# smolGura/fish-tts

Measured on AMD Instinct MI355X. Metric: semantic tokens/sec, higher is better.
Workload: dtype bf16; 1 GPU; openaudio-s1-mini shapes (BASELINE configs[1]): batch=1 per GPU, 48-token prompt, 215 frames (10 s), top-p sampling, hipGraph-captured frame step, + DAC codec decode; prompt_len=48, parallelism=replica x1, frame_engine=3

## Files before the change

fish-tts_amd/csrc/ar_kernels.h:

```cpp
#pragma once
#include "common.h"

namespace ft {

enum { PRO_NONE = 0, PRO_RMSNORM = 1 };
enum { EPI_STORE = 0, EPI_RESID = 1, EPI_SWIGLU = 2 };

__device__ __host__ __forceinline__ size_t xo_index(int m, int k, int ldm) { return ((size_t)(k >> 3) * ldm + m) * 8 + (k & 7); }

struct GemvP {
    const void* W;
    const void* bias;
    const float* x;
    int ldx;
    const void* gain;
    float eps;
    float* out;
    int ldo;
    const float* resid;
    int ldr;
    int N, K;
    int pro, epi;
    int nt;
};
// ... 1416 lines not shown
        const float* qrow = nullptr;
        if (p.noise && nfv < p.noise_rows) qrow = p.noise + (size_t)nfv * p.noise_row_len + p.noise_off;
        float q4[4];
        draw_noise4(p, ctl, qrow, i0, nfv, m, V, q4);
        ArgMax best{-1.f, 0x7fffffff};
#pragma unroll
        for (int e = 0; e < 4; ++e) {
            if (i0 + e < V) {
                const float prob = keep[e] ? rb<ROUND>(et[e] / Z2) : 0.f;
                best = better(best, ArgMax{rb<ROUND>(prob / rb<ROUND>(q4[e])), i0 + e});
            }
        }
        winner = block_best(best).i;
    }
    __syncthreads();
    finish_draw<WT>(p, m, winner, nfv);
}

struct SampCut {
    unsigned kstar;
    int nk;
    int all_kept;
    int argmax;
    float Lmax, Mt, Z2, Tc;
};

struct SampBigP {
    SampP s;
    SampCut* cut;
    int* chunk_cnt;
    float* part_score;
    int* part_idx;
    int nchunk;
};

__device__ __forceinline__ float key16_value(unsigned k16) {
    const uint32_t k = k16 << 16;
    const uint32_t u = (k & 0x80000000u) ? (k & 0x7fffffffu) : ~(k | 0xffffu);
    return __uint_as_float(u);
}

constexpr int SAMP_TH_THREADS = 1024;
constexpr int SAMP_TH_ROW = 33;
constexpr int SAMP_TH_OVF = 8;
constexpr size_t SAMP_TH_LDS = (size_t)SAMP_TH_THREADS * SAMP_TH_ROW * 4;

struct SampThShared {
    float red[16];
    int redi[16];
    float wsum[16];
    int wact[16];
    int AL[1024];
    unsigned ovf_key[SAMP_TH_OVF];
    unsigned ovf_cnt[SAMP_TH_OVF];
    int ovf_n;
    SampCut cut_s;
};

__device__ __forceinline__ void samp_cut_from_image(const SampBigP& b, const int m, const uint32_t* cimg, SampThShared& sh,
                                                    const bool has, const int kmax_t) {
    const SampP& p = b.s;
    const int tid = threadIdx.x, lane = tid & 63, wave = tid >> 6;
    const RowCtl ctl = p.ctl[m];
    float* red = sh.red;
    int* redi = sh.redi;
    float* wsum = sh.wsum;
    int* wact = sh.wact;
    int* AL = sh.AL;
    unsigned* ovf_key = sh.ovf_key;
    unsigned* ovf_cnt = sh.ovf_cnt;
    int& ovf_n = sh.ovf_n;
    SampCut& cut_s = sh.cut_s;
    const unsigned long long hb = __ballot(has);
    if (lane == 0) wact[wave] = __popcll(hb);
    __syncthreads();
    int abase = 0, n_active = 0;
    for (int w = 0; w < 16; ++w) { if (w < wave) abase += wact[w]; n_active += wact[w]; }
    if (has) AL[abase + __popcll(hb & ((1ull << lane) - 1ull))] = tid;
    ArgMax km = block_argmax(ArgMax{(float)kmax_t, tid}, red, redi);
    const unsigned kmax = (unsigned)(int)km.v;
    const float Lmax = key16_value(kmax);
    const int n_items = n_active * 64;
    const int ipt = (n_items + 1023) / 1024;
    const int i0 = tid * ipt, i1 = min(i0 + ipt, n_items);
    auto item_count = [&](int i, unsigned& k) -> float {
        const int g = AL[i >> 6], j = i & 63;
        k = 64u * g + j;
        const uint32_t w = cimg[g * SAMP_TH_ROW + (j >> 1)];
        unsigned c = (j & 1) ? (w >> 16) : (w & 0xffffu);
        if (c == 65535u)
            for (int q = 0; q < ovf_n && q < SAMP_TH_OVF; ++q) if (ovf_key[q] == k) c = ovf_cnt[q];
        return (float)c;
    };
    float z = 0.f;
    for (int i = i0; i < i1; ++i) {
        unsigned k;
        const float c = item_count(i, k);
        if (c > 0.f) z = fmaf(c, expf(key16_value(k) - Lmax), z);
    }
    const float Z = block_sum(z, red);
    const float tp = round_bf16(ctl.top_p);
    auto removed = [&](float cum) { return round_bf16(cum) > tp; };
    auto prob = [&](unsigned k16) { return round_bf16(expf(key16_value(k16) - Lmax) / Z); };
    float mt = 0.f;
    for (int i = i0; i < i1; ++i) {
        unsigned k;
        const float c = item_count(i, k);
        if (c > 0.f) mt = fmaf(c, prob(k), mt);
    }
    float suf = mt;
#pragma unroll
    for (int o = 1; o < 64; o <<= 1) {
        const float t = __shfl_down(suf, o, 64);
        if (lane + o < 64) suf += t;
    }
    __syncthreads();
    if (lane == 0) wsum[wave] = suf;
    __syncthreads();
    float above = suf - mt;
    for (int w = wave + 1; w < 16; ++w) above += wsum[w];
    int found = -1;
    unsigned f_key = 0;
    float f_above = 0.f, f_cnt = 0.f;
    float run = above;
    for (int i = i1 - 1; i >= i0; --i) {
        unsigned k;
        const float c = item_count(i, k);
        if (c > 0.f) {
            const float nxt = fmaf(c, prob(k), run);
            if (found < 0 && removed(nxt)) { found = i; f_key = k; f_above = run; f_cnt = c; }
            run = nxt;
        }
    }
    ArgMax who = block_argmax(ArgMax{found >= 0 ? (float)tid : -1.f, tid}, red, redi);
    if (tid == 0) { cut_s.all_kept = who.v < 0.f ? 1 : 0; cut_s.kstar = 0; cut_s.nk = 0; }
    __syncthreads();
    if (who.v >= 0.f && tid == (int)who.v) {
        const float pk = prob(f_key);
        int lo_n = 0, hi_n = (int)f_cnt;
        while (lo_n < hi_n) {
            const int mid = (lo_n + hi_n + 1) >> 1;
            if (removed(fmaf((float)mid, pk, f_above))) hi_n = mid - 1; else lo_n = mid;
        }
        if (f_key == kmax && lo_n < 1) lo_n = 1;
        cut_s.kstar = f_key;
        cut_s.nk = lo_n;
    }
    __syncthreads();
    const unsigned kstar = cut_s.kstar;
    const int nk = cut_s.nk, all_kept = cut_s.all_kept;
    const float Tc = fmaxf(ctl.temperature, 1e-5f);
    const float Mt = round_bf16(Lmax / Tc);
    float z2 = 0.f;
    for (int i = i0; i < i1; ++i) {
        unsigned k;
        const float c = item_count(i, k);
        if (c > 0.f) {
            float n = 0.f;
            if (all_kept || k > kstar) n = c;
            else if (k == kstar) n = (float)nk;
            if (n > 0.f) z2 = fmaf(n, expf(round_bf16(key16_value(k) / Tc) - Mt), z2);
        }
    }
    const float Z2 = block_sum(z2, red);
    if (tid == 0) {
        SampCut o;
        o.kstar = kstar; o.nk = nk; o.all_kept = all_kept; o.argmax = 0;
        o.Lmax = Lmax; o.Mt = Mt; o.Z2 = Z2; o.Tc = Tc;
        b.cut[m] = o;
    }
}

static __global__ __launch_bounds__(1024) void samp_cut_kernel(SampBigP b) {
    extern __shared__ __attribute__((aligned(16))) uint32_t cimg[];
    __shared__ SampThShared sh;
    __shared__ int pen_id[32];
    __shared__ float pen_val[32];
    const SampP& p = b.s;
    const int m = blockIdx.x, tid = threadIdx.x;
    float* L = p.logits + (size_t)m * p.ldl;
    const int V = p.V;
    const RowCtl ctl = p.ctl[m];
    const int nfv = p.nf[m];
    const int R = p.ncb + 1;
    const int* seq = p.seq + (size_t)m * R * p.cap;
    for (int i = tid; i < SAMP_TH_THREADS * SAMP_TH_ROW; i += 1024) cimg[i] = 0u;
    if (tid == 0) sh.ovf_n = 0;
    const int npen = nfv > 0 ? (p.cb == 0 ? R : 16) : 0;
    auto count1 = [&](float v) {
        const unsigned k = order_key(v) >> 16;
        atomicAdd(&cimg[(k >> 6) * SAMP_TH_ROW + ((k & 63u) >> 1)], (k & 1u) ? 0x10000u : 1u);
    };
    {
        if (nfv > 0) {
            const int it = nfv - 1;
            const int ws = it < 16 ? 0 : it - 16;
            if (tid < npen) {
                const int id = p.cb == 0 ? seq[(size_t)tid * p.cap + ws + 1] : seq[(size_t)(p.cb + 1) * p.cap + ws + 1 + tid];
                pen_id[tid] = -1;
                if (id >= 0 && id < V) {
                    const float sv = L[id];
                    pen_id[tid] = id;
                    pen_val[tid] = sv < 0.f ? round_bf16(sv * ctl.rep) : round_bf16(sv / ctl.rep);
                }
            }
            __syncthreads();
            if (tid < npen && pen_id[tid] >= 0) L[pen_id[tid]] = pen_val[tid];
        }
        if (p.cb == 0 && ctl.ban_eos && tid == 0 && p.im_end < V) L[p.im_end] = -INFINITY;
        __syncthreads();
        const int V16 = ((reinterpret_cast<uintptr_t>(L) & 15) == 0) ? (V / 16384) * 16384 : 0;
        float4 fa[4], fb[4];
        auto ld16 = [&](float4 (&f)[4], int base) {
#pragma unroll
            for (int u = 0; u < 4; ++u) f[u] = *reinterpret_cast<const float4*>(L + base + u * 4096 + tid * 4);
        };
        auto cnt16 = [&](const float4 (&f)[4]) {
#pragma unroll
            for (int u = 0; u < 4; ++u) { count1(f[u].x); count1(f[u].y); count1(f[u].z); count1(f[u].w); }
        };
        if (V16 > 0) ld16(fa, 0);
        for (int base = 0; base < V16; base += 32768) {
            if (base + 16384 < V16) ld16(fb, base + 16384);
            cnt16(fa);
            if (base + 32768 < V16) ld16(fa, base + 32768);
            if (base + 16384 < V16) cnt16(fb);
        }
        for (int base = V16; base < V; base += 4096) {
            float f[4];
#pragma unroll
            for (int u = 0; u < 4; ++u) { const int i = base + u * 1024 + tid; f[u] = i < V ? L[i] : 0.f; }
#pragma unroll
            for (int u = 0; u < 4; ++u) if (base + u * 1024 + tid < V) count1(f[u]);
        }
    }
    __syncthreads();
    const uint32_t* row = cimg + tid * SAMP_TH_ROW;
    int kmax_t = -1;
    unsigned tot = 0;
#pragma unroll 8
    for (int j = 0; j < 32; ++j) {
        const uint32_t w = row[j];
        const unsigned c0 = w & 0xffffu, c1 = w >> 16;
        if (c0) kmax_t = 64 * tid + 2 * j;
        if (c1) kmax_t = 64 * tid + 2 * j + 1;
        tot += c0 + c1;
    }
    const int total = (int)block_sum((float)tot, sh.red);
    if (total != V) {
        __shared__ unsigned exc_key[SAMP_TH_OVF];
        __shared__ unsigned exc_cnt[SAMP_TH_OVF];
        for (int i = tid; i < SAMP_TH_THREADS * SAMP_TH_ROW; i += 1024) cimg[i] = 0u;
        if (tid < SAMP_TH_OVF) { exc_key[tid] = 0xffffffffu; exc_cnt[tid] = 0u; }
        __syncthreads();
        for (int i = tid; i < V; i += 1024) {
            const unsigned k = order_key(L[i]) >> 16;
            uint32_t* d = &cimg[(k >> 6) * SAMP_TH_ROW + ((k & 63u) >> 1)];
            const unsigned shft = (k & 1u) * 16u;
            for (;;) {
                const uint32_t old = *reinterpret_cast<volatile uint32_t*>(d);
                if (((old >> shft) & 0xffffu) == 65535u) {
                    for (int q = 0; q < SAMP_TH_OVF; ++q) {
                        const unsigned prev = atomicCAS(&exc_key[q], 0xffffffffu, k);
                        if (prev == 0xffffffffu || prev == k) { atomicAdd(&exc_cnt[q], 1u); break; }
                    }
                    break;
                }
                if (atomicCAS(d, old, old + (1u << shft)) == old) break;
            }
        }
        __syncthreads();
        if (tid == 0) {
            int n = 0;
            for (int q = 0; q < SAMP_TH_OVF; ++q)
                if (exc_key[q] != 0xffffffffu) { sh.ovf_key[n] = exc_key[q]; sh.ovf_cnt[n] = 65535u + exc_cnt[q]; ++n; }
            sh.ovf_n = n;
        }
        kmax_t = -1;
        tot = 0;
        for (int j = 0; j < 32; ++j) {
            const uint32_t w = row[j];
            if (w & 0xffffu) kmax_t = 64 * tid + 2 * j;
            if (w >> 16) kmax_t = 64 * tid + 2 * j + 1;
            tot += (w & 0xffffu) + (w >> 16);
        }
        __syncthreads();
    }
    samp_cut_from_image(b, m, cimg, sh, tot != 0u, kmax_t);
}

static __global__ __launch_bounds__(256) void samp_count_kernel(SampBigP b) {
    __shared__ float red[4];
    const SampP& p = b.s;
    const int m = blockIdx.y, tid = threadIdx.x;
    const int c0 = blockIdx.x * 1024;
    const float* L = p.logits + (size_t)m * p.ldl;
    const SampCut cut = b.cut[m];
    float c = 0.f;
#pragma unroll
    for (int e = 0; e < 4; ++e) {
        const int i = c0 + 4 * tid + e;
        if (i < p.V && (order_key(L[i]) >> 16) == cut.kstar) c += 1.f;
    }
    c = wave_sum(c);
    if ((tid & 63) == 0) red[tid >> 6] = c;
    __syncthreads();
    if (tid == 0) b.chunk_cnt[(size_t)m * b.nchunk + blockIdx.x] = (int)(red[0] + red[1] + red[2] + red[3]);
}

static __global__ __launch_bounds__(256) void samp_race_kernel(SampBigP b) {
    __shared__ float red[4];
    __shared__ int redi[4];
    __shared__ int wcnt[4];
    const SampP& p = b.s;
    const int m = blockIdx.y, tid = threadIdx.x, lane = tid & 63, wave = tid >> 6;
    const int c0 = blockIdx.x * 1024;
    const float* L = p.logits + (size_t)m * p.ldl;
    const int V = p.V;
    const RowCtl ctl = p.ctl[m];
    const int nfv = p.nf[m];
    const SampCut cut = b.cut[m];
    float basef = 0.f;
// ... 72 lines not shown
```

fish-tts_amd/csrc/engine.h:

```cpp
#pragma once
#include <hip/hip_runtime.h>

#include <map>
#include <string>
#include <vector>

#include "../../include/fishtts_hip.h"
#include "../../include/fishtts_hip_test.h"
#include "common.h"

namespace ft {
struct RowCtl;
struct SampCut;
struct EngLayer;
}

struct FtTensor {
    void* p = nullptr;
    std::vector<int64_t> shape;
    int dtype = FT_BF16;
    int64_t numel() const {
        int64_t n = 1;
        for (auto s : shape) n *= s;
        return n;
// ... 31 lines not shown
          *femb = nullptr, *xf = nullptr, *qkvf = nullptr, *gf = nullptr, *flog = nullptr, *part_o = nullptr,
          *part_ml = nullptr;
    int n_slots = 0, nsplit = 1, cap = 0, fastV = 0, y_ld = 0;
    int nsplit_max = 1;
    bool nsplit_fixed = false;
    float *pf_x = nullptr, *pf_qkv = nullptr, *pf_y = nullptr;
    ft::bf16_t *pf_xn = nullptr, *pf_ybf = nullptr, *pf_g = nullptr, *pf_qbf = nullptr;
    int4* pf_seqs = nullptr;
    int2* pf_rows = nullptr;
    ft::bf16_t *xo_x = nullptr, *xo_xf = nullptr, *xo_femb = nullptr, *xo_y = nullptr, *xo_g = nullptr;
    ft::bf16_t* wide_qkv0_tab = nullptr;
    int xo_ldm = 0;
    int xo_pair = 0;
    bool no_attn_wide = false;
    bool no_head_stream = false;
    bool no_pair = false;
    int wide_min = 5;
    bool wide_ok = false;
    bool prefill_v0 = false;
    int prefill_gemm_mode = 2;
    size_t cache_m_stride = 0, fcache_m_stride = 0;

    int *d_pos = nullptr, *d_tok = nullptr, *d_tokn = nullptr, *d_seq = nullptr, *d_nf = nullptr,
        *d_done = nullptr, *d_prompt = nullptr;
    ft::RowCtl* d_ctl = nullptr;
    int *h_pin = nullptr;
    float* noise = nullptr;
    long noise_rows = 0, noise_row_len = 0;

    ft::SampCut* samp_cut = nullptr;
    int* samp_chunk_cnt = nullptr;
    float* samp_part_score = nullptr;
    int* samp_part_idx = nullptr;

    bool eng_on = false;
    bool eng_fast_on = false;
    int eng_nb = 0;
    ft::EngLayer *eng_layers = nullptr, *eng_flayers = nullptr;
    unsigned *eng_gx = nullptr, *eng_gqkv = nullptr, *eng_gy = nullptr, *eng_gxb = nullptr, *eng_gg = nullptr;
    unsigned long long* eng_gpart = nullptr;
    unsigned* eng_fast_g = nullptr;
    unsigned* eng_ctl = nullptr;
    size_t eng_lds_slow = 0, eng_lds_fast = 0, eng_fast_words = 0, eng_pool_words = 0;
    bool eng_relay = true;
    void* eng_qkv0_tab = nullptr;
    bool eng_pair = false;
    bool xl_shape = false;
    bool eng_xl = false;
    std::string path_str;
    const void* eng_slow_fn = nullptr;
    const void* eng_fast_fn = nullptr;
    size_t eng_pool_bytes = 0, eng_gpart_bytes = 0, eng_fast_bytes = 0;
    bool eng_suspended = false;
    int eng_strikes = 0, eng_last_where = 0;
    bool eng_owner = false;
    std::string eng_why;

    std::map<int, hipGraphExec_t> graphs;
    std::map<int, int> graph_nodes;

    bool prof = false, prof_count_only = false;
    std::vector<hipEvent_t> prof_ev;
    int64_t prof_bytes = 0, prof_launches = 0;

    CodecState* codec = nullptr;
};
// ... 15 lines not shown
```

fish-tts_amd/csrc/engine.hip:

```cpp
#include "engine.h"
#include "ar_kernels.h"
#include "frame_engine.h"
#include "wide_kernels.h"
#include "codec_kernels.h"

#include <math.h>

#include <algorithm>
#include <mutex>
#include <stdio.h>
#include <stdlib.h>
#include <string.h>

using namespace ft;

static std::string g_create_err;
static void eng_release(ft_ctx* ctx);

ft_status ft_fail(ft_ctx* ctx, ft_status code, const std::string& msg) {
    if (ctx) ctx->err = msg; else g_create_err = msg;
    return code;
}

template <typename S, typename D>
// ... 157 lines not shown
        const size_t S = c.max_seq_len;
        FT_TRY(dmalloc(ctx, &ctx->pf_x, S * c.dim));
        FT_TRY(dmalloc(ctx, &ctx->pf_qkv, S * qkvN));
        FT_TRY(dmalloc(ctx, &ctx->pf_y, S * c.n_head * c.head_dim));
        FT_TRY(dmalloc(ctx, &ctx->pf_xn, S * c.dim));
        FT_TRY(dmalloc(ctx, &ctx->pf_ybf, S * c.n_head * c.head_dim));
        FT_TRY(dmalloc(ctx, &ctx->pf_g, S * c.intermediate_size));
        FT_TRY(dmalloc(ctx, &ctx->pf_qbf, S * c.n_head * c.head_dim));
        FT_TRY(dmalloc(ctx, &ctx->pf_seqs, M));
        FT_TRY(dmalloc(ctx, &ctx->pf_rows, S));
    }
    if (c.dtype == FT_F16 || !ctx->prefill_v0) {
        const int HD = c.n_head * c.head_dim, HDf = c.fast_n_head * c.fast_head_dim;
        ctx->wide_ok = !getenv("FT_NO_WIDE") && !c.fast_attention_qkv_bias && !c.fast_attention_o_bias && c.fast_dim == c.dim &&
                       wide_k_ok(c.dim) && wide_k_ok(HD) && wide_k_ok(c.intermediate_size) && wide_k_ok(HDf) && wide_k_ok(c.fast_intermediate_size) &&
                       qkvN % 32 == 0 && fqkvN % 32 == 0 && c.intermediate_size % 16 == 0 && c.fast_intermediate_size % 16 == 0 &&
                       c.dim % 16 == 0 && c.vocab_size % 32 == 0 && ctx->fastV % 16 == 0;
        if (ctx->wide_ok) {
            ctx->xo_pair = (int)((M + 15) / 16 * 16);
            ctx->no_pair = getenv("FT_NO_PAIR") != nullptr;
            ctx->no_attn_wide = getenv("FT_NO_ATTN_WIDE") != nullptr;
            ctx->no_head_stream = getenv("FT_NO_HEAD_STREAM") != nullptr;
            ctx->xo_ldm = 2 * ctx->xo_pair;
            const size_t P = ctx->xo_ldm;
            FT_TRY(dmalloc(ctx, &ctx->xo_x, P * c.dim));
            FT_TRY(dmalloc(ctx, &ctx->xo_xf, P * c.fast_dim));
            FT_TRY(dmalloc(ctx, &ctx->xo_femb, P * c.fast_dim));
            FT_TRY(dmalloc(ctx, &ctx->xo_y, P * (size_t)std::max(HD, HDf)));
            FT_TRY(dmalloc(ctx, &ctx->xo_g, P * (size_t)std::max(c.intermediate_size, c.fast_intermediate_size)));
        }
    }
    const size_t nchunk = ((size_t)c.vocab_size + 1023) / 1024;
    FT_TRY(dmalloc(ctx, &ctx->samp_cut, M));
    FT_TRY(dmalloc(ctx, &ctx->samp_chunk_cnt, M * nchunk));
    FT_TRY(dmalloc(ctx, &ctx->samp_part_score, M * nchunk));
    FT_TRY(dmalloc(ctx, &ctx->samp_part_idx, M * nchunk));
    FT_HIP(ctx, hipHostMalloc((void**)&ctx->h_pin, (3 * M + 8) * sizeof(int), hipHostMallocDefault));
    return FT_OK;
}

extern "C" ft_status ft_create(const ft_ar_config* ar, const ft_codec_config* codec, int32_t device, ft_ctx** out) {
    if (!out || (!ar && !codec)) return ft_fail(nullptr, FT_ERR_ARG, "ft_create: need a config and an out pointer");
    int ndev = 0;
    if (hipGetDeviceCount(&ndev) != hipSuccess || ndev == 0)
        return ft_fail(nullptr, FT_ERR_HIP, "ft_create: no HIP device visible (the MI355X path has no CPU fallback)");
    if (device < 0 || device >= ndev) return ft_fail(nullptr, FT_ERR_ARG, "ft_create: bad device index");
    ft_ctx* ctx = new ft_ctx();
    ctx->device = device;
    ft_status st = FT_OK;
    do {
        if (hipSetDevice(device) != hipSuccess) { st = ft_fail(ctx, FT_ERR_HIP, "hipSetDevice failed"); break; }
        if (hipStreamCreateWithFlags(&ctx->stream, hipStreamNonBlocking) != hipSuccess) {
            st = ft_fail(ctx, FT_ERR_HIP, "hipStreamCreate failed"); break;
        }
        if (ar) {
            ctx->c = *ar;
            ctx->has_ar = true;
            if ((st = ar_validate(ctx)) != FT_OK) break;
            if ((st = ar_alloc(ctx)) != FT_OK) break;
            ar_expected(ctx);
        }
        if (codec) {
            ctx->cc = *codec;
            ctx->has_codec = true;
            if ((st = codec_create(ctx)) != FT_OK) break;
            codec_expected(ctx);
// ... 893 lines not shown
    else { s.logits = ctx->flog + (size_t)m0 * ctx->fastV; s.ldl = ctx->fastV; s.V = ctx->fastV; }
    s.ctl = ctx->d_ctl + m0; s.tokn = ctx->d_tokn + (size_t)m0 * R; s.seq = ctx->d_seq + (size_t)m0 * R * ctx->cap;
    s.cap = ctx->cap; s.nf = ctx->d_nf + m0; s.cb = cb; s.ncb = c.num_codebooks; s.sem_begin = c.semantic_begin_id;
    s.im_end = c.im_end_id; s.cbsize = c.codebook_size; s.fast_emb = ctx->fast_emb;
    s.femb = ctx->femb + (size_t)m0 * c.fast_dim; s.Df = c.fast_dim; s.noise = ctx->noise;
    s.noise_row_len = ctx->noise_row_len; s.noise_rows = ctx->noise_rows;
    s.noise_off = cb == 0 ? 0 : (long)c.vocab_size + (long)(cb - 1) * ctx->fastV;
    s.last = last ? 1 : 0; s.tok = ctx->d_tok + (size_t)m0 * R; s.pos = ctx->d_pos + m0; s.done = ctx->d_done + m0;
    if (wide_batch(L)) {
        s.femb_xo = (cb == 0 && wide_pair(L) ? ctx->xo_x + (size_t)ctx->xo_pair * 8 : ctx->xo_femb) + (size_t)m0 * 8;
        s.femb_ldm = ctx->xo_ldm;
        what |= cb == 0 && wide_pair(L) ? DRAW_XO_PAIR : DRAW_XO_FEMB;
        if (cb >= 1 && cb + 1 < c.num_codebooks && ctx->wide_qkv0_tab) {
            what |= DRAW_QKV0_TAB;
            s.qkv0_tab = ctx->wide_qkv0_tab; s.qkv0_n = (c.fast_n_head + 2 * c.fast_n_local_heads) * c.fast_head_dim;
            s.qkv0_out = ctx->qkvf + (size_t)m0 * s.qkv0_n;
        }
    }
    if (s.V <= 1024) {
        sample_small_kernel<WT, ROUND><<<L.M, 256, 0, L.s>>>(s);
        what |= DRAW_SMALL;
    } else if (ROUND == RND_BF16) {
        SampBigP b{};
        b.s = s; b.nchunk = (s.V + 1023) / 1024;
        b.cut = ctx->samp_cut + m0;
        b.chunk_cnt = ctx->samp_chunk_cnt + (size_t)m0 * b.nchunk;
        b.part_score = ctx->samp_part_score + (size_t)m0 * b.nchunk;
        b.part_idx = ctx->samp_part_idx + (size_t)m0 * b.nchunk;
        const dim3 gridc(b.nchunk, L.M);
        {
            static DevOnce once;
            once.run([] {
                hipFuncSetAttribute((const void*)samp_cut_kernel, hipFuncAttributeMaxDynamicSharedMemorySize, (int)SAMP_TH_LDS);
            });
        }
        samp_cut_kernel<<<L.M, SAMP_TH_THREADS, SAMP_TH_LDS, L.s>>>(b);
        samp_count_kernel<<<gridc, 256, 0, L.s>>>(b);
        samp_race_kernel<<<gridc, 256, 0, L.s>>>(b);
        samp_finish_kernel<WT><<<L.M, 256, 0, L.s>>>(b);
        what |= DRAW_FOUR;
    } else {
        sample_block_kernel<WT, ROUND><<<L.M, 1024, 0, L.s>>>(s);
        what |= DRAW_BLOCK;
    }
    L.chk();
    return what;
}

template <typename WT, int ROUND>
static void enqueue_fast_step(Launch& L, const int cb, const bool pair = false) {
    ft_ctx* ctx = L.ctx;
    const ft_ar_config& c = ctx->c;
    const int m0 = L.m0;
    const int Df = c.fast_dim, Hf = c.fast_n_head, Hkvf = c.fast_n_local_heads, hdf = c.fast_head_dim;
    const size_t qkvN = (size_t)(Hf + 2 * Hkvf) * hdf;
    float* xf = ctx->xf + (size_t)m0 * Df;
    float* qkvf = ctx->qkvf + (size_t)m0 * qkvN;
    float* gf = ctx->gf + (size_t)m0 * c.fast_intermediate_size;
    {
        const float* xin = cb == 0 ? ctx->hid + (size_t)m0 * Df : ctx->femb + (size_t)m0 * Df;
        const bool wide = wide_batch(L);
        for (int li = 0; li < c.n_fast_layer; ++li) {
            const FtLayer& l = ctx->flayers[li];
            const float* xl = li == 0 ? xin : xf;
            if (wide) {
                if constexpr (ROUND != RND_NONE) {
                    const int HDf = Hf * hdf, Ff = c.fast_intermediate_size, M = L.M, ldm = ctx->xo_ldm;
                    const int rows = pair ? ctx->xo_pair + M : M;
                    const bf16_t* xin_o = ((cb == 0 || pair) ? ctx->xo_x : ctx->xo_femb) + (size_t)m0 * 8;
// ... 503 lines not shown
    ft_kv_snapshot* s = new ft_kv_snapshot();
    s->n_pos = n_pos;
    s->bytes = (size_t)c.n_layer * 2 * c.n_local_heads * n_pos * c.head_dim * ctx->esz;
    if (hipMalloc((void**)&s->data, s->bytes) != hipSuccess) {
        delete s;
        return ft_fail(ctx, FT_ERR_HIP, "ft_ar_kv_save: out of device memory");
    }
    ft_status st = kv_copy(ctx, s->data, n_pos, slot, true);
    if (st == FT_OK && hipStreamSynchronize(ctx->stream) != hipSuccess) st = ft_fail(ctx, FT_ERR_HIP, "ft_ar_kv_save: copy failed");
    if (st != FT_OK) { hipFree(s->data); delete s; return st; }
    *out = s;
    return FT_OK;
}

extern "C" ft_status ft_ar_kv_restore(ft_ctx* ctx, const ft_kv_snapshot* snap, int32_t slot) {
    FT_TRY(ar_ready(ctx));
    if (!snap || !snap->data) return ft_fail(ctx, FT_ERR_ARG, "ft_ar_kv_restore: null snapshot");
    if (slot < 0 || slot >= ctx->c.max_batch) return ft_fail(ctx, FT_ERR_ARG, "ft_ar_kv_restore: bad slot");
    if (snap->n_pos > ctx->n_slots) return ft_fail(ctx, FT_ERR_ARG, "ft_ar_kv_restore: snapshot longer than the cache");
    return kv_copy(ctx, snap->data, snap->n_pos, slot, false);
}

extern "C" int32_t ft_ar_kv_positions(const ft_kv_snapshot* snap) { return snap ? snap->n_pos : 0; }

extern "C" void ft_ar_kv_free(ft_ctx* ctx, ft_kv_snapshot* snap) {
    if (!snap) return;
    if (ctx) { hipSetDevice(ctx->device); hipStreamSynchronize(ctx->stream); }
    if (snap->data) hipFree(snap->data);
    delete snap;
}

static int graph_key(const ft_ctx* ctx, int M, int frames) {
    const bool eng = M == 1 && (ctx->eng_on || ctx->eng_fast_on) && !ctx->eng_suspended;
    return (M * 64 + ctx->nsplit) + (frames > 1 ? frames * (1 << 20) : 0) + (eng ? (1 << 28) : 0);
}

static ft_status get_graph(ft_ctx* ctx, int M, hipGraphExec_t* out, int frames = 1) {
    const int key = graph_key(ctx, M, frames);
    auto it = ctx->graphs.find(key);
    if (it != ctx->graphs.end()) { *out = it->second; return FT_OK; }
    const int R = ctx->c.num_codebooks + 1;
    hipGraph_t graph = nullptr;
    FT_HIP(ctx, hipStreamBeginCapture(ctx->stream, hipStreamCaptureModeThreadLocal));
    Launch L{ctx, ctx->stream, 0, M, 0};
    for (int f = 0; f < frames; ++f) enqueue_frame(L, ctx->d_tok, 1, R, 0);
    hipError_t e = hipStreamEndCapture(ctx->stream, &graph);
    if (L.err != hipSuccess) e = L.err;
    if (e != hipSuccess) {
        if (graph) hipGraphDestroy(graph);
        return ft_fail(ctx, FT_ERR_HIP, std::string("graph capture: ") + hipGetErrorString(e));
    }
    hipGraphExec_t exec = nullptr;
    { size_t nn = 0; if (frames == 1 && hipGraphGetNodes(graph, nullptr, &nn) == hipSuccess) ctx->graph_nodes[key] = (int)nn; }
    e = hipGraphInstantiate(&exec, graph, nullptr, nullptr, 0);
    hipGraphDestroy(graph);
    if (e != hipSuccess) return ft_fail(ctx, FT_ERR_HIP, std::string("graph instantiate: ") + hipGetErrorString(e));
    ctx->graphs[key] = exec;
    *out = exec;
    return FT_OK;
}

extern "C" ft_status ft_ar_decode(ft_ctx* ctx, int32_t nslots, int32_t n_frames, const ft_sampling* sp,
                                  int32_t poll, int32_t* out_frames, int32_t* out_n) {
    FT_TRY(ar_ready(ctx));
    const ft_ar_config& c = ctx->c;
    if (!sp || !out_frames || !out_n) return ft_fail(ctx, FT_ERR_ARG, "ft_ar_decode: null argument");
    if (nslots < 1 || nslots > c.max_batch) return ft_fail(ctx, FT_ERR_ARG, "ft_ar_decode: bad nslots");
// ... 122 lines not shown
    FT_HIP(ctx, hipMemcpyAsync(ctx->eng_ctl + ENG_CTL_EPOCH, &epoch, sizeof epoch, hipMemcpyHostToDevice, ctx->stream));
    if (ctx->eng_gx) FT_HIP(ctx, hipMemsetAsync(ctx->eng_gx, 0, ctx->eng_pool_bytes, ctx->stream));
    if (ctx->eng_gpart) FT_HIP(ctx, hipMemsetAsync(ctx->eng_gpart, 0, ctx->eng_gpart_bytes, ctx->stream));
    if (ctx->eng_fast_g) FT_HIP(ctx, hipMemsetAsync(ctx->eng_fast_g, 0, ctx->eng_fast_bytes, ctx->stream));
    FT_HIP(ctx, hipStreamSynchronize(ctx->stream));
    char buf[256];
    if (ctx->eng_strikes >= ENG_MAX_STRIKES) {
        for (auto it = ctx->graphs.begin(); it != ctx->graphs.end();) {
            if (it->first & (1 << 28)) { hipGraphExecDestroy(it->second); it = ctx->graphs.erase(it); } else ++it;
        }
        eng_release(ctx);
        snprintf(buf, sizeof buf, "launch path: the frame engine was turned off after %d hand-off time-outs (last in phase %u)",
                 ctx->eng_strikes, w[ENG_CTL_WHERE]);
        ctx->eng_why = buf;
    }
    fprintf(stderr, "fish_tts_amd: frame engine: a hand-off timed out (phase %u, strike %d of %d): the frames are redone on the "
            "launch path%s\n", w[ENG_CTL_WHERE], ctx->eng_strikes, ENG_MAX_STRIKES,
            ctx->eng_strikes >= ENG_MAX_STRIKES ? "; the engine stays off for this context" : "");
    return FT_OK;
}
static bool eng_in_use(const ft_ctx* ctx) { return (ctx->eng_on || ctx->eng_fast_on) && !ctx->eng_suspended; }

extern "C" ft_status ft_ar_engine_state(ft_ctx* ctx, int32_t* flags, int32_t* aborted, int32_t* where) {
    FT_TRY(ar_ready(ctx));
    if (flags) *flags = (ctx->eng_on ? 1 : 0) | (ctx->eng_fast_on ? 2 : 0);
    if (aborted) *aborted = ctx->eng_strikes;
    if (where) *where = ctx->eng_last_where;
    return FT_OK;
}

extern "C" const char* ft_ar_frame_path(const ft_ctx* ctx) {
    if (!ctx) return "";
    ft_ctx* c = const_cast<ft_ctx*>(ctx);
    c->path_str = ctx->eng_why + (ctx->wide_ok
                                      ? "; lock-step batches of >= 5 rows: MFMA launches with fused row operations (five per layer)"
                                      : "; lock-step batches: multi-row GEMV launches");
    return c->path_str.c_str();
}

extern "C" ft_status ft_test_engine_fault(ft_ctx* ctx, int32_t which, int32_t wg, int32_t skip) {
    FT_TRY(ar_ready(ctx));
    if (!ctx->eng_ctl || !(which == 0 ? ctx->eng_on : ctx->eng_fast_on)) return ft_fail(ctx, FT_ERR_STATE, "ft_test_engine_fault: the frame engine is off");
    if (wg < 0 || wg >= ctx->eng_nb || skip < 0) return ft_fail(ctx, FT_ERR_ARG, "ft_test_engine_fault: bad workgroup or skip count");
    const unsigned v[2] = {(which == 0 ? 0u : ENG_FAULT_FAST) + 1u + (unsigned)wg, (unsigned)skip};
    static_assert(ENG_CTL_FAULT_SKIP == ENG_CTL_FAULT + 1, "the two words are written by one copy");
    FT_HIP(ctx, hipStreamSynchronize(ctx->stream));
    FT_HIP(ctx, hipMemcpy(ctx->eng_ctl + ENG_CTL_FAULT, v, sizeof v, hipMemcpyHostToDevice));
    return FT_OK;
}

extern "C" ft_status ft_test_ar_attn_plan(ft_ctx* ctx, int32_t* nsplit, int32_t* xl, int32_t* n_slots) {
    FT_TRY(ar_ready(ctx));
    if (nsplit) *nsplit = ctx->nsplit;
    if (xl) *xl = ctx->eng_on && ctx->eng_xl ? 1 : 0;
    if (n_slots) *n_slots = ctx->n_slots;
    return FT_OK;
}

extern "C" ft_status ft_ar_park(ft_ctx* ctx, int32_t slot) {
    FT_TRY(ar_ready(ctx));
    const ft_ar_config& c = ctx->c;
    if (slot < 0 || slot >= c.max_batch) return ft_fail(ctx, FT_ERR_ARG, "ft_ar_park: bad slot");
    const int R = c.num_codebooks + 1;
    FT_TRY(ft_ar_reset(ctx, slot));
    int* h = ctx->h_pin;
    h[0] = c.im_end_id; h[1] = 1;
    FT_HIP(ctx, hipMemcpyAsync(ctx->d_seq + (size_t)slot * R * ctx->cap, h, sizeof(int), hipMemcpyHostToDevice, ctx->stream));
    FT_HIP(ctx, hipMemcpyAsync(ctx->d_nf + slot, h + 1, sizeof(int), hipMemcpyHostToDevice, ctx->stream));
    FT_HIP(ctx, hipMemcpyAsync(ctx->d_done + slot, h + 1, sizeof(int), hipMemcpyHostToDevice, ctx->stream));
// ... 968 lines not shown
```

Before: 787.2 tokens/s.

## Cache top-p cut classes in registers and rework the histogram image layout in samp_cut

Rewrites the semantic-token top-p cut kernel so that each thread's histogram classes (keys, counts, exp values) are loaded once into registers and reused across the Z, cumulative-mass, search and Z2 passes. It also bins raw float bits directly with a padded word index instead of computing order_key, and fuses the per-group count, active-flag and max reductions into one wave-level pass. The previous kernel is kept behind FT_CUT_PLAIN and timestamp hooks are added. This trades more register pressure and extra complexity (reversed scan for negative values, an overflow fallback path) for fewer LDS rereads and fewer barriers.

```diff
diff --git a/fish-tts_amd/csrc/ar_kernels.h b/fish-tts_amd/csrc/ar_kernels.h
--- a/fish-tts_amd/csrc/ar_kernels.h
+++ b/fish-tts_amd/csrc/ar_kernels.h
@@ -1472,6 +1472,7 @@
     float* part_score;
     int* part_idx;
     int nchunk;
+    unsigned long long* stamps;
 };
 
 __device__ __forceinline__ float key16_value(unsigned k16) {
@@ -1497,7 +1498,9 @@
     SampCut cut_s;
 };
 
-__device__ __forceinline__ void samp_cut_from_image(const SampBigP& b, const int m, const uint32_t* cimg, SampThShared& sh,
+#define SAMP_STAMP(k) do { if (b.stamps && threadIdx.x == 0) b.stamps[(size_t)blockIdx.x * 16 + (k)] = __builtin_amdgcn_s_memrealtime(); } while (0)
+
+__device__ __forceinline__ void samp_cut_from_image_plain(const SampBigP& b, const int m, const uint32_t* cimg, SampThShared& sh,
                                                     const bool has, const int kmax_t) {
     const SampP& p = b.s;
     const int tid = threadIdx.x, lane = tid & 63, wave = tid >> 6;
@@ -1518,6 +1521,7 @@
     for (int w = 0; w < 16; ++w) { if (w < wave) abase += wact[w]; n_active += wact[w]; }
     if (has) AL[abase + __popcll(hb & ((1ull << lane) - 1ull))] = tid;
     ArgMax km = block_argmax(ArgMax{(float)kmax_t, tid}, red, redi);
+    SAMP_STAMP(4);
     const unsigned kmax = (unsigned)(int)km.v;
     const float Lmax = key16_value(kmax);
     const int n_items = n_active * 64;
@@ -1539,6 +1543,7 @@
         if (c > 0.f) z = fmaf(c, expf(key16_value(k) - Lmax), z);
     }
     const float Z = block_sum(z, red);
+    SAMP_STAMP(5);
     const float tp = round_bf16(ctl.top_p);
     auto removed = [&](float cum) { return round_bf16(cum) > tp; };
     auto prob = [&](unsigned k16) { return round_bf16(expf(key16_value(k16) - Lmax) / Z); };
@@ -1559,6 +1564,7 @@
     __syncthreads();
     float above = suf - mt;
     for (int w = wave + 1; w < 16; ++w) above += wsum[w];
+    SAMP_STAMP(6);
     int found = -1;
     unsigned f_key = 0;
     float f_above = 0.f, f_cnt = 0.f;
@@ -1573,6 +1579,7 @@
         }
     }
     ArgMax who = block_argmax(ArgMax{found >= 0 ? (float)tid : -1.f, tid}, red, redi);
+    SAMP_STAMP(7);
     if (tid == 0) { cut_s.all_kept = who.v < 0.f ? 1 : 0; cut_s.kstar = 0; cut_s.nk = 0; }
     __syncthreads();
     if (who.v >= 0.f && tid == (int)who.v) {
@@ -1587,6 +1594,7 @@
         cut_s.nk = lo_n;
     }
     __syncthreads();
+    SAMP_STAMP(8);
     const unsigned kstar = cut_s.kstar;
     const int nk = cut_s.nk, all_kept = cut_s.all_kept;
     const float Tc = fmaxf(ctl.temperature, 1e-5f);
@@ -1603,21 +1611,24 @@
         }
     }
     const float Z2 = block_sum(z2, red);
+    SAMP_STAMP(9);
     if (tid == 0) {
         SampCut o;
         o.kstar = kstar; o.nk = nk; o.all_kept = all_kept; o.argmax = 0;
         o.Lmax = Lmax; o.Mt = Mt; o.Z2 = Z2; o.Tc = Tc;
         b.cut[m] = o;
     }
-}
-
-static __global__ __launch_bounds__(1024) void samp_cut_kernel(SampBigP b) {
+    SAMP_STAMP(10);
+}
+
+static __global__ __launch_bounds__(1024) void samp_cut_plain_kernel(SampBigP b) {
     extern __shared__ __attribute__((aligned(16))) uint32_t cimg[];
     __shared__ SampThShared sh;
     __shared__ int pen_id[32];
     __shared__ float pen_val[32];
     const SampP& p = b.s;
     const int m = blockIdx.x, tid = threadIdx.x;
+    SAMP_STAMP(0);
     float* L = p.logits + (size_t)m * p.ldl;
     const int V = p.V;
     const RowCtl ctl = p.ctl[m];
@@ -1649,6 +1660,7 @@
         }
         if (p.cb == 0 && ctl.ban_eos && tid == 0 && p.im_end < V) L[p.im_end] = -INFINITY;
         __syncthreads();
+        SAMP_STAMP(1);
         const int V16 = ((reinterpret_cast<uintptr_t>(L) & 15) == 0) ? (V / 16384) * 16384 : 0;
         float4 fa[4], fb[4];
         auto ld16 = [&](float4 (&f)[4], int base) {
@@ -1675,6 +1687,7 @@
         }
     }
     __syncthreads();
+    SAMP_STAMP(2);
     const uint32_t* row = cimg + tid * SAMP_TH_ROW;
     int kmax_t = -1;
     unsigned tot = 0;
@@ -1726,8 +1739,337 @@
         }
         __syncthreads();
     }
-    samp_cut_from_image(b, m, cimg, sh, tot != 0u, kmax_t);
-}
+    SAMP_STAMP(3);
+    samp_cut_from_image_plain(b, m, cimg, sh, tot != 0u, kmax_t);
+}
+
+
+constexpr int SAMP_IPT_REG = 8;
+
+template <int RAW>
+__device__ __forceinline__ unsigned samp_img_h(unsigned k) {
+    if (RAW) return (k & 0x8000u) ? (k & 0x7fffu) : (~k & 0xffffu);
+    return k;
+}
+__device__ __forceinline__ unsigned samp_img_word(unsigned h) { return (h >> 1) + (h >> 6); }
+
+template <int RAW>
+__device__ __forceinline__ void samp_cut_from_image(const SampBigP& b, const int m, const uint32_t* cimg, SampThShared& sh,
+                                                    const int n_active, const unsigned kmax) {
+    const SampP& p = b.s;
+    const int tid = threadIdx.x, lane = tid & 63, wave = tid >> 6;
+    const RowCtl ctl = p.ctl[m];
+    float* red = sh.red;
+    int* redi = sh.redi;
+    float* wsum = sh.wsum;
+    int* AL = sh.AL;
+    unsigned* ovf_key = sh.ovf_key;
+    unsigned* ovf_cnt = sh.ovf_cnt;
+    int& ovf_n = sh.ovf_n;
+    SampCut& cut_s = sh.cut_s;
+    const float Lmax = key16_value(kmax);
+    const int n_items = n_active * 64;
+    const int ipt = (n_items + 1023) / 1024;
+    const int i0 = tid * ipt, i1 = min(i0 + ipt, n_items);
+    const bool in_regs = ipt <= SAMP_IPT_REG;
+    auto item_count = [&](int i, unsigned& k) -> float {
+        const int g = AL[i >> 6], j = i & 63;
+        k = 64u * g + j;
+        const unsigned h = samp_img_h<RAW>(k);
+        const uint32_t w = cimg[samp_img_word(h)];
+        unsigned c = (h & 1u) ? (w >> 16) : (w & 0xffffu);
+        if (c == 65535u)
+            for (int q = 0; q < ovf_n && q < SAMP_TH_OVF; ++q) if (ovf_key[q] == k) c = ovf_cnt[q];
+        return (float)c;
+    };
+    unsigned kk[SAMP_IPT_REG];
+    float cc[SAMP_IPT_REG], ev[SAMP_IPT_REG];
+    float z = 0.f;
+    if (in_regs) {
+#pragma unroll
+        for (int u = 0; u < SAMP_IPT_REG; ++u) {
+            kk[u] = 0u; cc[u] = 0.f; ev[u] = 0.f;
+            if (i0 + u < i1) cc[u] = item_count(i0 + u, kk[u]);
+        }
+#pragma unroll
+        for (int u = 0; u < SAMP_IPT_REG; ++u)
+            if (cc[u] > 0.f) { ev[u] = expf(key16_value(kk[u]) - Lmax); z = fmaf(cc[u], ev[u], z); }
+    } else {
+        for (int i = i0; i < i1; ++i) {
+            unsigned k;
+            const float c = item_count(i, k);
+            if (c > 0.f) z = fmaf(c, expf(key16_value(k) - Lmax), z);
+        }
+    }
+    const float Z = block_sum(z, red);
+    SAMP_STAMP(5);
+    const float tp = round_bf16(ctl.top_p);
+    auto removed = [&](float cum) { return round_bf16(cum) > tp; };
+    auto prob = [&](unsigned k16) { return round_bf16(expf(key16_value(k16) - Lmax) / Z); };
+    float mt = 0.f;
+    if (in_regs) {
+#pragma unroll
+        for (int u = 0; u < SAMP_IPT_REG; ++u)
+            if (cc[u] > 0.f) { ev[u] = round_bf16(ev[u] / Z); mt = fmaf(cc[u], ev[u], mt); }
+    } else {
+        for (int i = i0; i < i1; ++i) {
+            unsigned k;
+            const float c = item_count(i, k);
+            if (c > 0.f) mt = fmaf(c, prob(k), mt);
+        }
+    }
+    float suf = mt;
+#pragma unroll
+    for (int o = 1; o < 64; o <<= 1) {
+        const float t = __shfl_down(suf, o, 64);
+        if (lane + o < 64) suf += t;
+    }
+    __syncthreads();
+    if (lane == 0) wsum[wave] = suf;
+    __syncthreads();
+    float above = suf - mt;
+    for (int w = wave + 1; w < 16; ++w) above += wsum[w];
+    SAMP_STAMP(6);
+    int found = -1;
+    unsigned f_key = 0;
+    float f_above = 0.f, f_cnt = 0.f, f_pr = 0.f;
+    float run = above;
+    if (in_regs) {
+#pragma unroll
+        for (int u = SAMP_IPT_REG - 1; u >= 0; --u) {
+            if (cc[u] > 0.f) {
+                const float nxt = fmaf(cc[u], ev[u], run);
+                if (found < 0 && removed(nxt)) { found = i0 + u; f_key = kk[u]; f_above = run; f_cnt = cc[u]; f_pr = ev[u]; }
+                run = nxt;
+            }
+        }
+    } else {
+        for (int i = i1 - 1; i >= i0; --i) {
+            unsigned k;
+            const float c = item_count(i, k);
+            if (c > 0.f) {
+                const float pr = prob(k);
+                const float nxt = fmaf(c, pr, run);
+                if (found < 0 && removed(nxt)) { found = i; f_key = k; f_above = run; f_cnt = c; f_pr = pr; }
+                run = nxt;
+            }
+        }
+    }
+    ArgMax who = block_argmax(ArgMax{found >= 0 ? (float)tid : -1.f, tid}, red, redi);
+    SAMP_STAMP(7);
+    const bool cut_found = who.v >= 0.f;
+    if (cut_found && tid == (int)who.v) {
+        const float pk = f_pr;
+        int lo_n = 0, hi_n = (int)f_cnt;
+        while (lo_n < hi_n) {
+            const int mid = (lo_n + hi_n + 1) >> 1;
+            if (removed(fmaf((float)mid, pk, f_above))) hi_n = mid - 1; else lo_n = mid;
+        }
+        if (f_key == kmax && lo_n < 1) lo_n = 1;
+        cut_s.kstar = f_key;
+        cut_s.nk = lo_n;
+    }
+    __syncthreads();
+    SAMP_STAMP(8);
+    const unsigned kstar = cut_found ? cut_s.kstar : 0u;
+    const int nk = cut_found ? cut_s.nk : 0, all_kept = cut_found ? 0 : 1;
+    const float Tc = fmaxf(ctl.temperature, 1e-5f);
+    const float Mt = round_bf16(Lmax / Tc);
+    auto stay = [&](unsigned k, float c) { return (all_kept || k > kstar) ? c : k == kstar ? (float)nk : 0.f; };
+    float z2 = 0.f;
+    if (in_regs) {
+#pragma unroll
+        for (int u = 0; u < SAMP_IPT_REG; ++u) {
+            if (cc[u] > 0.f) {
+                const float n = stay(kk[u], cc[u]);
+                if (n > 0.f) z2 = fmaf(n, expf(round_bf16(key16_value(kk[u]) / Tc) - Mt), z2);
+            }
+        }
+    } else {
+        for (int i = i0; i < i1; ++i) {
+            unsigned k;
+            const float c = item_count(i, k);
+            if (c > 0.f) {
+                const float n = stay(k, c);
+                if (n > 0.f) z2 = fmaf(n, expf(round_bf16(key16_value(k) / Tc) - Mt), z2);
+            }
+        }
+    }
+    const float Z2 = block_sum(z2, red);
+    SAMP_STAMP(9);
+    if (tid == 0) {
+        SampCut o;
+        o.kstar = kstar; o.nk = nk; o.all_kept = all_kept; o.argmax = 0;
+        o.Lmax = Lmax; o.Mt = Mt; o.Z2 = Z2; o.Tc = Tc;
+        b.cut[m] = o;
+    }
+    SAMP_STAMP(10);
+}
+
+template <int RAW>
+__device__ __forceinline__ void samp_cut_row(const SampBigP& b) {
+    extern __shared__ __attribute__((aligned(16))) uint32_t cimg[];
+    __shared__ SampThShared sh;
+    __shared__ int pen_id[32];
+    __shared__ float pen_val[32];
+    const SampP& p = b.s;
+    const int m = blockIdx.x, tid = threadIdx.x;
+    SAMP_STAMP(0);
+    float* L = p.logits + (size_t)m * p.ldl;
+    const int V = p.V;
+    const RowCtl ctl = p.ctl[m];
+    const int nfv = p.nf[m];
+    const int R = p.ncb + 1;
+    const int* seq = p.seq + (size_t)m * R * p.cap;
+    for (int i = tid; i < SAMP_TH_THREADS * SAMP_TH_ROW; i += 1024) cimg[i] = 0u;
+    if (tid == 0) sh.ovf_n = 0;
+    const int npen = nfv > 0 ? (p.cb == 0 ? R : 16) : 0;
+    auto count1 = [&](float v) {
+        if (RAW) {
+            const uint32_t u = __float_as_uint(v);
+            atomicAdd(&cimg[(u >> 17) + (u >> 22)], max(u & 0x10000u, 1u));
+        } else {
+            const unsigned k = order_key(v) >> 16;
+            atomicAdd(&cimg[samp_img_word(k)], (k & 1u) ? 0x10000u : 1u);
+        }
+    };
+    {
+        if (nfv > 0) {
+            const int it = nfv - 1;
+            const int ws = it < 16 ? 0 : it - 16;
+            if (tid < npen) {
+                const int id = p.cb == 0 ? seq[(size_t)tid * p.cap + ws + 1] : seq[(size_t)(p.cb + 1) * p.cap + ws + 1 + tid];
+                pen_id[tid] = -1;
+                if (id >= 0 && id < V) {
+                    const float sv = L[id];
+                    pen_id[tid] = id;
+                    pen_val[tid] = sv < 0.f ? round_bf16(sv * ctl.rep) : round_bf16(sv / ctl.rep);
+                }
+            }
+            __syncthreads();
+            if (tid < npen && pen_id[tid] >= 0) L[pen_id[tid]] = pen_val[tid];
+        }
+        if (p.cb == 0 && ctl.ban_eos && tid == 0 && p.im_end < V) L[p.im_end] = -INFINITY;
+        __syncthreads();
+        SAMP_STAMP(1);
+        const int V16 = ((reinterpret_cast<uintptr_t>(L) & 15) == 0) ? (V / 16384) * 16384 : 0;
+        float4 fa[4], fb[4];
+        auto ld16 = [&](float4 (&f)[4], int base) {
+#pragma unroll
+            for (int u = 0; u < 4; ++u) f[u] = *reinterpret_cast<const float4*>(L + base + u * 4096 + tid * 4);
+        };
+        auto cnt16 = [&](const float4 (&f)[4]) {
+#pragma unroll
+            for (int u = 0; u < 4; ++u) { count1(f[u].x); count1(f[u].y); count1(f[u].z); count1(f[u].w); }
+        };
+        if (V16 > 0) ld16(fa, 0);
+        for (int base = 0; base < V16; base += 32768) {
+            if (base + 16384 < V16) ld16(fb, base + 16384);
+            cnt16(fa);
+            if (base + 32768 < V16) ld16(fa, base + 32768);
+            if (base + 16384 < V16) cnt16(fb);
+        }
+        for (int base = V16; base < V; base += 4096) {
+            float f[4];
+#pragma unroll
+            for (int u = 0; u < 4; ++u) { const int i = base + u * 1024 + tid; f[u] = i < V ? L[i] : 0.f; }
+#pragma unroll
+            for (int u = 0; u < 4; ++u) if (base + u * 1024 + tid < V) count1(f[u]);
+        }
+    }
+    __syncthreads();
+    SAMP_STAMP(2);
+    const int lane = tid & 63, wave = tid >> 6;
+    const bool rev = RAW && tid < 512;
+    const uint32_t* row = cimg + (RAW ? (rev ? 1023 - tid : tid - 512) : tid) * SAMP_TH_ROW;
+    int kmax_t = -1;
+    unsigned tot = 0;
+    auto scan_group = [&]() {
+        int kj = -1;
+        tot = 0;
+        if (rev) {
+#pragma unroll 8
+            for (int j = 0; j < 32; ++j) {
+                const uint32_t w = row[31 - j];
+                tot = __builtin_amdgcn_sad_u16(w, 0u, tot);
+                if (w) kj = j;
+            }
+        } else {
+#pragma unroll 8
+            for (int j = 0; j < 32; ++j) {
+                const uint32_t w = row[j];
+                tot = __builtin_amdgcn_sad_u16(w, 0u, tot);
+                if (w) kj = j;
+            }
+        }
+        kmax_t = -1;
+        if (kj >= 0) {
+            const uint32_t w = row[rev ? 31 - kj : kj];
+            kmax_t = 64 * tid + 2 * kj + ((rev ? w & 0xffffu : w >> 16) ? 1 : 0);
+        }
+    };
+    int total = 0, abase = 0, n_active = 0, kmax = -1;
+    unsigned long long hb = 0ull;
+    auto reduce_groups = [&]() {
+        hb = __ballot(tot != 0u);
+        const float tw = wave_sum((float)tot);
+        const ArgMax kw = wave_argmax(ArgMax{(float)kmax_t, tid});
+        if (lane == 0) { sh.red[wave] = tw; sh.wact[wave] = __popcll(hb); sh.redi[wave] = (int)kw.v; }
+        __syncthreads();
+        float t = 0.f;
+        abase = 0; n_active = 0; kmax = -1;
+        for (int w = 0; w < 16; ++w) {
+            t += sh.red[w];
+            if (w < wave) abase += sh.wact[w];
+            n_active += sh.wact[w];
+            kmax = max(kmax, sh.redi[w]);
+        }
+        total = (int)t;
+    };
+    scan_group();
+    reduce_groups();
+    if (total != V) {
+        __shared__ unsigned exc_key[SAMP_TH_OVF];
+        __shared__ unsigned exc_cnt[SAMP_TH_OVF];
+        for (int i = tid; i < SAMP_TH_THREADS * SAMP_TH_ROW; i += 1024) cimg[i] = 0u;
+        if (tid < SAMP_TH_OVF) { exc_key[tid] = 0xffffffffu; exc_cnt[tid] = 0u; }
+        __syncthreads();
+        for (int i = tid; i < V; i += 1024) {
+            const unsigned k = order_key(L[i]) >> 16;
+            const unsigned h = samp_img_h<RAW>(k);
+            uint32_t* d = &cimg[samp_img_word(h)];
+            const unsigned shft = (h & 1u) * 16u;
+            for (;;) {
+                const uint32_t old = *reinterpret_cast<volatile uint32_t*>(d);
+                if (((old >> shft) & 0xffffu) == 65535u) {
+                    for (int q = 0; q < SAMP_TH_OVF; ++q) {
+                        const unsigned prev = atomicCAS(&exc_key[q], 0xffffffffu, k);
+                        if (prev == 0xffffffffu || prev == k) { atomicAdd(&exc_cnt[q], 1u); break; }
+                    }
+                    break;
+                }
+                if (atomicCAS(d, old, old + (1u << shft)) == old) break;
+            }
+        }
+        __syncthreads();
+        if (tid == 0) {
+            int n = 0;
+            for (int q = 0; q < SAMP_TH_OVF; ++q)
+                if (exc_key[q] != 0xffffffffu) { sh.ovf_key[n] = exc_key[q]; sh.ovf_cnt[n] = 65535u + exc_cnt[q]; ++n; }
+            sh.ovf_n = n;
+        }
+        scan_group();
+        reduce_groups();
+    }
+    SAMP_STAMP(3);
+    if (tot != 0u) sh.AL[abase + __popcll(hb & ((1ull << lane) - 1ull))] = tid;
+    __syncthreads();
+    SAMP_STAMP(4);
+    samp_cut_from_image<RAW>(b, m, cimg, sh, n_active, (unsigned)kmax);
+}
+
+static __global__ __launch_bounds__(1024) void samp_cut_kernel(SampBigP b) { samp_cut_row<1>(b); }
+#undef SAMP_STAMP
 
 static __global__ __launch_bounds__(256) void samp_count_kernel(SampBigP b) {
     __shared__ float red[4];
diff --git a/fish-tts_amd/csrc/engine.h b/fish-tts_amd/csrc/engine.h
--- a/fish-tts_amd/csrc/engine.h
+++ b/fish-tts_amd/csrc/engine.h
@@ -87,6 +87,7 @@
     int* samp_chunk_cnt = nullptr;
     float* samp_part_score = nullptr;
     int* samp_part_idx = nullptr;
+    bool cut_plain = false;
 
     bool eng_on = false;
     bool eng_fast_on = false;
diff --git a/fish-tts_amd/csrc/engine.hip b/fish-tts_amd/csrc/engine.hip
--- a/fish-tts_amd/csrc/engine.hip
+++ b/fish-tts_amd/csrc/engine.hip
@@ -213,6 +213,7 @@
     }
     const size_t nchunk = ((size_t)c.vocab_size + 1023) / 1024;
     FT_TRY(dmalloc(ctx, &ctx->samp_cut, M));
+    { const char* cp = getenv("FT_CUT_PLAIN"); ctx->cut_plain = cp != nullptr && cp[0] != '\0' && cp[0] != '0'; }
     FT_TRY(dmalloc(ctx, &ctx->samp_chunk_cnt, M * nchunk));
     FT_TRY(dmalloc(ctx, &ctx->samp_part_score, M * nchunk));
     FT_TRY(dmalloc(ctx, &ctx->samp_part_idx, M * nchunk));
@@ -1172,9 +1173,11 @@
             static DevOnce once;
             once.run([] {
                 hipFuncSetAttribute((const void*)samp_cut_kernel, hipFuncAttributeMaxDynamicSharedMemorySize, (int)SAMP_TH_LDS);
+                hipFuncSetAttribute((const void*)samp_cut_plain_kernel, hipFuncAttributeMaxDynamicSharedMemorySize, (int)SAMP_TH_LDS);
             });
         }
-        samp_cut_kernel<<<L.M, SAMP_TH_THREADS, SAMP_TH_LDS, L.s>>>(b);
+        if (ctx->cut_plain) samp_cut_plain_kernel<<<L.M, SAMP_TH_THREADS, SAMP_TH_LDS, L.s>>>(b);
+        else samp_cut_kernel<<<L.M, SAMP_TH_THREADS, SAMP_TH_LDS, L.s>>>(b);
         samp_count_kernel<<<gridc, 256, 0, L.s>>>(b);
         samp_race_kernel<<<gridc, 256, 0, L.s>>>(b);
         samp_finish_kernel<WT><<<L.M, 256, 0, L.s>>>(b);
@@ -1744,7 +1747,7 @@
 
 static int graph_key(const ft_ctx* ctx, int M, int frames) {
     const bool eng = M == 1 && (ctx->eng_on || ctx->eng_fast_on) && !ctx->eng_suspended;
-    return (M * 64 + ctx->nsplit) + (frames > 1 ? frames * (1 << 20) : 0) + (eng ? (1 << 28) : 0);
+    return (M * 64 + ctx->nsplit) + (frames > 1 ? frames * (1 << 20) : 0) + (eng ? (1 << 28) : 0) + (ctx->cut_plain ? (1 << 29) : 0);
 }
 
 static ft_status get_graph(ft_ctx* ctx, int M, hipGraphExec_t* out, int frames = 1) {
@@ -1933,9 +1936,10 @@
 extern "C" const char* ft_ar_frame_path(const ft_ctx* ctx) {
     if (!ctx) return "";
     ft_ctx* c = const_cast<ft_ctx*>(ctx);
-    c->path_str = ctx->eng_why + (ctx->wide_ok
-                                      ? "; lock-step batches of >= 5 rows: MFMA launches with fused row operations (five per layer)"
-                                      : "; lock-step batches: multi-row GEMV launches");
+    c->path_str = ctx->eng_why + (ctx->cut_plain ? "; semantic draw: samp_cut in its plain form (FT_CUT_PLAIN is set)"
+                                                 : "; semantic draw: samp_cut searches on classes cached in registers") +
+                  (ctx->wide_ok ? "; lock-step batches of >= 5 rows: MFMA launches with fused row operations (five per layer)"
+                                : "; lock-step batches: multi-row GEMV launches");
     return c->path_str.c_str();
 }
 
```

Result: no change. 793.0 tokens/s (median of 6 runs) (+0.7%).
